# xiaoyi018/VAE-Var

Hardware: AMD Instinct MI355X
Metric: 4D-Var inner-loop iters/sec + wall-clock to convergence, 69ch 128×256 state (higher is better)
Workload: dtype f32 (GEMMs: fp16x3 split, fp32-level error)

## Files before the change

include/vaevar.h:

```cpp
#ifndef VAEVAR_H
#define VAEVAR_H
#include <stdint.h>

#ifdef __cplusplus
extern "C" {
#endif

#define VV_E_ARG 1001
#define VV_E_STATE 1002
#define VV_E_ALLOC 1003

typedef struct vv_ctx vv_ctx;

#define VV_ARCH_LGUNET 0
#define VV_ARCH_LGUNET1 1

typedef struct vv_lgunet_config {
  int img_size[2];
  int patch_size[2];
  int stride[2];
  int n_groups;
  int inchans[8];
  int outchans[8];
  int enc_dim;
// ... 150 lines not shown
int vv_profile_start(vv_ctx* ctx);
int vv_profile_stop(vv_ctx* ctx, double* ms, double* flops, double* bytes, int* launches, int ncls);

int vv_nearest_map(int in_size, int out_size, int* map);

#define VV_GEMM_F32 0
#define VV_GEMM_SPLIT 1
#define VV_GEMM_SPLIT16 2
int vv_set_gemm_math(vv_ctx* ctx, int math);
int vv_get_gemm_math(vv_ctx* ctx, int* math);

int vv_set_tuning(vv_ctx* ctx, const char* key, int value);
int vv_get_tuning(vv_ctx* ctx, const char* key, int* value);
int vv_set_debug_sync(int enable);

int vv_gemm_register_weight(vv_ctx* ctx, const float* B, int N, int K);

int vv_attention_global(vv_ctx* ctx, const float* qkv, float* out, int N, int C, int heads, void* stream);

int vv_gemm(vv_ctx* ctx, int M, int N, int K, const float* A, const float* B, const float* bias, float* C,
            int tile, void* stream);
int vv_gemm_epi(vv_ctx* ctx, int M, int N, int K, const float* A, const float* B, const float* bias, float* C,
                float* aux, int epi, int tile, void* stream);
int vv_gelu_eval(vv_ctx* ctx, const float* x, float* y, float* dy, int64_t n, int form, void* stream);

#ifdef __cplusplus
}
#endif
#endif
```

vae-var_amd/csrc/vv_engine.hip:

```cpp
#include <hip/hip_runtime.h>

#include <sys/prctl.h>
#include <time.h>

#include <algorithm>
#include <array>
#include <atomic>
#include <chrono>
#include <cmath>
#include <cstdarg>
#include <cstdio>
#include <cstdlib>
#include <cstring>
#include <memory>
#include <optional>
#include <string>
#include <unordered_map>
#include <vector>

#include "../../include/vaevar.h"
#include "vv_api.h"
#include "vv_fcst.h"
#include "vv_kernels.h"

// ... 909 lines not shown
  l.gamma = g.gamma;
  l.eps = ln.eps;
  l.pl = g.pl;
  l.rs = g.rs;
  l.stats = g.stats;
  if (bwd) {
    l.bwd = 1;
    l.lmap = ln.map;
    l.x = g.x;
    l.res = g.res;
    l.y = g.y;
  } else {
    l.gmap = ln.map;
    l.ginv = ginv;
    l.lo_x = ln.map ? 0 : 1;
    l.beta = g.beta;
  }
  return vv::gemm_ln_applies(a, l, sc.ws);
}

int gemm_layernorm(const GemmArgs& a, const LnArgs& ln, bool bwd, const int* ginv, const Scratch& sc, hipStream_t st) {
  vv::GemmLnArgs l;
  if (fixup_ln_applies(a, ln, bwd, ginv, sc, l)) {
    CK(vv::gemm_ln(a, l, st, sc.ws));
    return 0;
  }
  CK(gemm_nt(a, st, -1, sc.ws));
  CK(bwd ? layernorm_bwd(ln, st) : layernorm_fwd(ln, st));
  return 0;
}

int gemm_into_block(const GemmArgs& a, const Blk* n, const Scratch& sc, hipStream_t st, bool& ln1_ran) {
  ln1_ran = n && !ablk_fused(n->S, sc, n->ws, false);
  if (!ln1_ran) {
    CK(gemm_nt(a, st, -1, sc.ws));
    return 0;
  }
  const int* ginv = vv::tuning_of(sc.tune).fixup_ln_rows ? n->idxinv() : nullptr;
  return gemm_layernorm(a, block_ln(*n, 1, qkv_gemm(*n).apre != nullptr), false, ginv, sc, st);
}

int attn_half_fwd(const Blk& k, bool ln1_ran, const LnArgs* ln2, hipStream_t st) {
  const Scratch& sc = k.sc;
  vv::AblkArgs aa;
  if (ablk_fused(k.S, sc, k.ws, false) && ablk_args(k, nullptr, aa)) {
    CK(vv::ablk_fwd(aa, st));
// ... 849 lines not shown
        g.exec = nullptr;
        g.eager_only = true;
        (void)hipGetLastError();
        (void)fail(r ? r : (int)(ec != hipSuccess ? ec : ei), "closure graph capture failed (%s); eager launches",
                   hipGetErrorString(ec != hipSuccess ? ec : ei));
        const int r2 = closure_enqueue(ctx, P.Z, gz, nullptr, st);
        if (r2) return r2;
      }
    }
    if (g.exec) {
      VV_HIP(hipGraphLaunch(g.exec, st));
      ++g.launches;
    }
  }
  if (grad_z) VV_HIP(hipMemcpyAsync(grad_z, P.GZ, P.zn * sizeof(float), hipMemcpyDeviceToDevice, st));
  if (d_J) VV_HIP(hipMemcpyAsync(d_J, P.dJ, 2 * P.B * sizeof(double), hipMemcpyDeviceToDevice, st));
  return 0;
}

}

extern "C" {

int vv_version(void) { return 113; }

int vv_last_error(char* buf, int cap) {
  if (!buf || cap <= 0) return VV_E_ARG;
  snprintf(buf, cap, "%s", g_err.c_str());
  return 0;
}

int vv_lgunet_param_count(const vv_lgunet_config* cfg, int* count) {
  if (cfg && cfg->arch == VV_ARCH_LGUNET1) {
    std::vector<vvf::ParamInfo> v;
    std::string err;
    const int r = vvf::params(cfg, v, err);
    if (r) return fail(r, "%s", err.c_str());
    *count = (int)v.size();
    return 0;
  }
  Cfg c;
  int r = parse_cfg(cfg, c);
  if (r) return r;
  *count = (int)enumerate_params(c).size();
  return 0;
}

// ... 773 lines not shown
  if (!f) return fail(VV_E_ARG, "unknown tuning key '%s'", key ? key : "(null)");
  *value = *f;
  return 0;
}

int vv_set_debug_sync(int enable) {
  g_sync_check.store(enable ? 1 : 0, std::memory_order_relaxed);
  return 0;
}

int vv_set_closure_graph(vv_ctx* ctx, int enable) {
  if (!ctx) return fail(VV_E_ARG, "null context");
  int r = set_dev(ctx);
  if (r) return r;
  drop_graphs(ctx);
  memo_clear(ctx);
  ctx->use_graphs = enable != 0;
  return 0;
}

int vv_get_counter(const char* name, long long* value) {
  if (!name || !value) return fail(VV_E_ARG, "null argument");
  static const char* names[vv::CNT_N] = {"rowsplit", "fixup_ln", "splitk_fixup", "gather_scales", "h5_split",
                                          "closure_recall_hit", "closure_recall_miss"};
  for (int c = 0; c < vv::CNT_N; ++c)
    if (!strcmp(name, names[c])) {
      *value = vv::launch_count(c);
      return 0;
    }
  return fail(VV_E_ARG, "unknown counter '%s'", name);
}

int vv_get_closure_graph(vv_ctx* ctx, int kind, long long* info) {
  if (!ctx || !info || kind < 0 || kind > 1) return fail(VV_E_ARG, "null context / info or kind not 0 / 1");
  const auto& g = ctx->graphs[kind];
  info[0] = ctx->use_graphs ? 1 : 0;
  info[1] = g.exec ? 1 : 0;
  info[2] = g.eager_only ? 1 : 0;
  info[3] = g.launches;
  return 0;
}

int vv_get_gemm_math(vv_ctx* ctx, int* math) {
  if (!ctx || !math) return fail(VV_E_ARG, "null argument");
  *math = ctx->math;
  return 0;
}
// ... 86 lines not shown
  if (epi != EPI_STORE && epi != EPI_GELU && epi != EPI_DGELU) return fail(VV_E_ARG, "epilogue %d", epi);
  if (epi == EPI_DGELU && !aux) return fail(VV_E_ARG, "EPI_DGELU reads the pre-activation aux");
  int r = set_dev(ctx);
  if (r) return r;
  GemmArgs a = vv::gemm_args(M, N, K, 1, epi, ctx->math, &ctx->tune);
  a.g[0] = {A, nullptr, B, bias, C, nullptr, aux};
  if (ctx->math == vv::GEMM_SPLIT16) {
    VV_HIP(grow(ctx->apl, ctx->apl_halfs, (size_t)M * 2 * K, sizeof(unsigned short), (hipStream_t)stream, true));
    a.apl = ctx->apl;
    a.apl_halfs = ctx->apl_halfs;
  }
  VV_HIP(vv::gemm_nt(a, (hipStream_t)stream, tile, ctx->gemm_ws));
  return 0;
}

int vv_gemm(vv_ctx* ctx, int M, int N, int K, const float* A, const float* B, const float* bias, float* C, int tile,
            void* stream) {
  return gemm_entry(ctx, M, N, K, A, B, bias, C, nullptr, EPI_STORE, tile, stream);
}

int vv_gemm_epi(vv_ctx* ctx, int M, int N, int K, const float* A, const float* B, const float* bias, float* C,
                float* aux, int epi, int tile, void* stream) {
  return gemm_entry(ctx, M, N, K, A, B, bias, C, aux, epi, tile, stream);
}

int vv_gelu_eval(vv_ctx* ctx, const float* x, float* y, float* dy, int64_t n, int form, void* stream) {
  if (!ctx || !x || !y || !dy || n < 0 || (form != 0 && form != 1)) return fail(VV_E_ARG, "bad argument");
  int r = set_dev(ctx);
  if (r) return r;
  VV_HIP(vv::gelu_eval(x, y, dy, n, form, (hipStream_t)stream));
  return 0;
}

int vv_attention_global(vv_ctx* ctx, const float* qkv, float* out, int N, int C, int heads, void* stream) {
  if (!ctx || !qkv || !out) return fail(VV_E_ARG, "null argument");
  if (N <= 0 || !vv::gattn_supported(C, heads))
    return fail(VV_E_ARG, "global attention needs N > 0 and head_dim 64, 96, 128 or 192 (N %d, C %d, heads %d)", N, C,
                heads);
  int r = set_dev(ctx);
  if (r) return r;
  VV_HIP(grow(ctx->gattn_ws, ctx->gattn_bytes, vv::gattn_ws_bytes(N, C, heads), 1, (hipStream_t)stream, true));
  VV_HIP(vv::gattn(qkv, out, C, N, C, heads, ctx->gattn_ws, (hipStream_t)stream, ctx->tune.gattn_qf));
  return 0;
}

int vv_sc4dvar_bind(vv_ctx* ctx, int flow_model_id, int T, int C, int Hs, int Ws, const float* xb, const float* yo,
// ... 148 lines not shown
```

vae-var_amd/csrc/vv_gemm.hip:

```cpp
#include "vv_gelu.h"
#include "vv_kernels.h"
#include "vv_lanes.h"

#include <algorithm>
#include <cmath>
#include <cstdlib>
#include <cstring>
#include <mutex>
#include <type_traits>
#include <utility>
#include <vector>

namespace vv {

typedef float f4 __attribute__((ext_vector_type(4)));
typedef float f16v __attribute__((ext_vector_type(16)));

__device__ __forceinline__ float gelu_f(float x) { return gelu_fast(x); }
__device__ __forceinline__ float dgelu_f(float x) { return dgelu_fast(x); }

constexpr int KALIGN = 32;

hipError_t set_lds_limit(const void* k, size_t lds) {
  static std::mutex mu;
// ... 7 lines not shown
  done.emplace_back(k, dev);
  return hipSuccess;
}

int device_cus() {
  static std::mutex mu;
  static int cus[64] = {0};
  int dev = 0;
  if (hipGetDevice(&dev) != hipSuccess || dev < 0 || dev >= 64) return 256;
  std::lock_guard<std::mutex> lk(mu);
  if (!cus[dev]) {
    hipDeviceProp_t p;
    cus[dev] = (hipGetDeviceProperties(&p, dev) == hipSuccess && p.multiProcessorCount > 0) ? p.multiProcessorCount : 256;
  }
  return cus[dev];
}

struct TileShape {
  int id, bm, bn, wm, wn;
};
constexpr TileShape kTiles[] = {{0, 128, 128, 2, 2},  {2, 64, 64, 2, 2},    {4, 32, 64, 1, 2},    {24, 64, 64, 2, 2},
                                {25, 128, 64, 2, 2},  {26, 64, 64, 2, 2},   {27, 64, 64, 2, 2},   {34, 128, 128, 2, 2},
                                {36, 128, 128, 2, 2}, {44, 256, 128, 4, 2}, {46, 128, 128, 2, 2}, {47, 256, 128, 4, 2},
                                {48, 256, 128, 4, 2}, {49, 256, 144, 4, 2}};
constexpr const TileShape* tile_shape(int t) {
  for (const TileShape& s : kTiles)
    if (s.id == t) return &s;
  return nullptr;
}
bool valid_tile(int t) { return tile_shape(t) != nullptr; }

struct LaunchPlan {
  int T, tail;
  dim3 grid;
};
static LaunchPlan launch_plan(const GemmArgs& a, int bm, int bn) {
  const int T = ((a.N + bn - 1) / bn) * ((a.M + bm - 1) / bm);
  const int tail = a.tsplit > 1 ? T - a.tdp : 0;
  return {T, tail, dim3(tail ? a.tdp + tail * a.tsplit : T, 1, a.ngroups)};
}

template <class F>
static hipError_t with_epi(int epi, F&& f) {
  switch (epi) {
    case EPI_STORE: return f(std::integral_constant<int, EPI_STORE>{});
    case EPI_GELU: return f(std::integral_constant<int, EPI_GELU>{});
    case EPI_RESID: return f(std::integral_constant<int, EPI_RESID>{});
// ... 2056 lines not shown
static hipError_t launch_h3(const GemmArgs& a, hipStream_t s) {
  constexpr TileShape S = *tile_shape(TILE);
  constexpr int BM = S.bm;
  static_assert(S.bn == 128 && S.wm == BM / 64 && S.wn == 2, "k_gemm_h3 / k_gemm_h3m's tile");
  if (a.K % 32 || a.ksplit % 32) return hipErrorInvalidValue;
  if (!h3_ready(a)) return hipErrorInvalidValue;
  const float* sc = a.ws + kWsFloats;
  if (a.ascale_phys && !a.arow)
    sc = a.ascale;
  else if (a.ascale_phys)
    hipLaunchKernelGGL(k_gather_scales, dim3((a.M + 255) / 256, 1, a.ngroups), dim3(256), 0, s, a.ascale, a.arow,
                       const_cast<float*>(sc), a.M);
  else
    launch_rowscale(a, const_cast<float*>(sc), s);
  const size_t lds = 2 * (2 * (S.bm + S.bn) * 32) * sizeof(unsigned short);
  const LaunchPlan p = launch_plan(a, S.bm, S.bn);
  return with_epi(a.epi, [&](auto E) {
    constexpr int EPI = decltype(E)::value;
    return MF == 16 ? launch_h3m_k<EPI, BM>(a, s, p.grid, lds, p.tail, sc)
                    : launch_h3_k<EPI, BM>(a, s, p.grid, lds, p.tail, sc);
  });
}

static bool h3_tile(int t) { return t == 36 || t == 44 || t == 46 || t == 47 || t == 48 || t == 49; }
bool gemm_plane_tile(int t) { return t == 48 || t == 49; }
int* tuning_field(Tuning& t, const char* key) {
  if (!key) return nullptr;
#define VV_KNOB(name, def, ok) \
  if (!std::strcmp(key, #name)) return &t.name;
#include "vv_tuning.def"
  return nullptr;
}
bool tuning_value_ok(const char* key, int v) {
#define VV_KNOB(name, def, ok) \
  if (key && !std::strcmp(key, #name)) return ok;
#include "vv_tuning.def"
  return v == 0 || v == 1;
}

static hipError_t launch_variant(int t, const GemmArgs& a, hipStream_t s) {
  switch (t) {
    case 0: return launch_tile<0>(a, s);
    case 2: return launch_tile<2>(a, s);
    case 4: return launch_tile<4>(a, s);
    case 24: return launch_bs<24, 2>(a, s);
    case 25: return launch_bs<25, 2>(a, s);
    case 26: return launch_bs<26, 3>(a, s);
    case 27: return launch_bs<27, 1>(a, s);
    case 34: return launch_bs2(a, s);
    case 36: return launch_h3<36, 32>(a, s);
    case 44: return launch_h3<44, 32>(a, s);
    case 46: return launch_h3<46, 16>(a, s);
    case 47: return launch_h3<47, 16>(a, s);
    case 48: return launch_h4(a, s);
    case 49: return launch_h4(a, s, true);
    default: return hipErrorInvalidValue;
  }
}

static long tiles_of(const GemmArgs& a, int bm, int bn) {
  return (long)((a.M + bm - 1) / bm) * ((a.N + bn - 1) / bn) * a.ngroups;
}

struct SplitArena {
  const float* base;
  size_t n;
  const unsigned short* planes;
};
static std::vector<SplitArena> g_split;

static size_t split16_scale_off(size_t n) { return (10 * n + 255) & ~size_t(255); }
size_t split_arena_bytes(size_t n) { return split16_scale_off(n) + (n / 32 + 1) * sizeof(float); }

void register_split_arena(const float* base, size_t n, const unsigned short* planes) {
  unregister_split_arena(base);
  g_split.push_back({base, n, planes});
}
void unregister_split_arena(const float* base) {
// ... 106 lines not shown
  if (tiles_of(a, 64, 64) >= 512) return 2;
  return 4;
}

static int group_m(const GemmArgs& a, const TileShape& sh) {
  const int ntm = (a.M + sh.bm - 1) / sh.bm, ntn = (a.N + sh.bn - 1) / sh.bn;
  const double tx = (double)ntm * ntn / 8.0;
  return std::max(1, std::min(ntm, (int)std::lround(std::sqrt(tx * sh.bn / sh.bm))));
}

static int resolve_tile(GemmArgs& a, int tile_hint) {
  int t = tile_hint >= 0 ? tile_hint : pick_tile(a);
  if (!valid_tile(t)) return -1;
  const Tuning& TU = tuning_of(a.tune);
  if (tile_hint < 0 && TU.h4 && a.math == GEMM_SPLIT16 &&
      (t == 44 || t == 47 || (t == 36 && tiles_of(a, 256, 128) >= (TU.h4_small ? 64 : 144))))
    t = 48;
  for (int g = 0; g < a.ngroups; ++g) {
    a.g[g].Bh = nullptr;
    a.g[g].Bs = nullptr;
    if (h3_tile(t) && (!a.ldb || a.ldb == a.K)) split16_of(a.g[g].B, a.K, a.g[g].Bh, a.g[g].Bs);
  }
  if (h3_tile(t) && !h3_ready(a)) t = 34;
  if ((t == 48 || t == 49) && !h4_ready(a)) t = 47;
  if (t == 48 && tile_hint < 0 && TU.h5 && a.N % 144 == 0) {
    const long P = device_cus(), t48 = tiles_of(a, 256, 128), t49 = tiles_of(a, 256, 144);
    if (t48 % P != 0 && t49 % P == 0) t = 49;
  }
  return t;
}

int gemm_tile_of(const GemmArgs& a_in, int tile_hint) {
  GemmArgs a = a_in;
  if (!a.ws) a.ws = reinterpret_cast<float*>(1);
  return resolve_tile(a, tile_hint);
}

static hipError_t gemm_prepare(GemmArgs& a, int tile_hint, float* ws, int& t) {
  if (a.M <= 0 || a.N <= 0 || a.ngroups <= 0 || a.ngroups > kMaxGroups) return hipErrorInvalidValue;
  if (a.K % KALIGN != 0 || a.ksplit % KALIGN != 0 || a.ksplit <= 0 || a.ksplit > a.K) return hipErrorInvalidValue;
  if ((a.lda & 3) || (a.lda2 & 3) || (a.K & 3) || (a.ldb & 3) || (a.ldb && a.ldb < a.K)) return hipErrorInvalidValue;
  if (a.apre && (!a.ascale || a.g[0].A2)) return hipErrorInvalidValue;
  const int num_cu = device_cus();
  a.tdp = 0;
  a.tsplit = 1;
  a.ws = ws;
  a.ascale_phys = 0;
  const Tuning& TU = tuning_of(a.tune);
  if (a.ascale && TU.ln_scales) {
    bool ok = true;
    for (int g = 0; g < a.ngroups; ++g) ok = ok && !a.g[g].A2;
    a.ascale_phys = ok ? 1 : 0;
  }
  t = resolve_tile(a, tile_hint);
  if (t < 0) return hipErrorInvalidValue;
  if (a.apre && !gemm_plane_tile(t)) return hipErrorInvalidValue;
  if (a.opl && (!gemm_plane_tile(t) || (a.epi != EPI_GELU && a.epi != EPI_DGELU) || a.ngroups != 1 || a.crow || a.N % 32 ||
                !a.ors || !a.obw))
    return hipErrorInvalidValue;
  for (int g = 0; g < a.ngroups; ++g) {
    a.g[g].Bp = (t >= 21 && (!a.ldb || a.ldb == a.K)) ? split_planes_of(a.g[g].B) : nullptr;
    a.g[g].Ap = (t >= 21 && t < 36 && !a.g[g].A2 && !a.g[g].Ap) ? split_planes_exact(a.g[g].A) : a.g[g].Ap;
  }
  const TileShape& sh = *tile_shape(t);
  a.gm = group_m(a, sh);
  if (ws && a.ngroups == 1) {
    const int T = launch_plan(a, sh.bm, sh.bn).T;
    const size_t tile_f = (size_t)sh.bm * sh.bn;
    const int P = num_cu, nkt = a.K / 32;
    const int tdp = (T / P) * P, tail = T - tdp;
    if (tdp > 0 && tail > 0 && tail <= P / 2 && t != 49) {
      const int tail_minkt = std::max(1, TU.tail_minkt);
      int S = std::min(P / tail, nkt / tail_minkt);
      while (S > 1 && (size_t)tail * S * tile_f > kWsFloats) --S;
      if (S > 1) {
        a.tdp = tdp;
        a.tsplit = S;
      }
    } else if (tdp == 0 && h3_tile(t) && t != 49 && TU.small_split) {
      const int min_kt = std::max(1, t == 48 ? TU.h4_split_minkt : TU.small_split_minkt);
      int S = std::min(((t == 36 || t == 46 ? 2 : 1) * P) / T, nkt / min_kt);
      while (S > 1 && (size_t)T * S * tile_f > kWsFloats) --S;
      if (S > 1) a.tsplit = S;
    }
  }
  return hipSuccess;
}

static bool apply_h5_split(GemmArgs& a, int& t, bool ok) {
  const TileShape& sh = *tile_shape(49);
  const long P = device_cus(), T49 = tiles_of(a, sh.bm, sh.bn);
  if (!ok || !tuning_of(a.tune).h5_split || t != 48 || a.ngroups != 1 || a.N % sh.bn != 0 || a.N % 128 != 0 ||
      T49 <= 0 || P % T49 != 0 || P / T49 < 2 || P / T49 > 4 || (size_t)P * sh.bm * sh.bn > kWsFloats ||
      a.K / 32 < P / T49)
    return false;
  t = 49;
  a.tsplit = (int)(P / T49);
  a.nofix = 1;
  a.gm = group_m(a, sh);
  return true;
}

hipError_t gemm_nt(const GemmArgs& a_in, hipStream_t s, int tile_hint, float* ws) {
  GemmArgs a = a_in;
  a.nofix = 0;
  a.t49 = 0;
  int t = -1;
  if (hipError_t e = gemm_prepare(a, tile_hint, ws, t)) return e;
  const bool fix49 = apply_h5_split(a, t, tile_hint < 0 && a.tsplit > 1 && a.tdp == 0 && !a.crow && !a.opl &&
                                              (a.epi == EPI_STORE || a.epi == EPI_RESID));
  const int ph = prof_begin(s);
  hipError_t e = launch_variant(t, a, s);
  if (e == hipSuccess && fix49) {
    count_launch(CNT_SPLITK_FIXUP);
    const dim3 grid(tiles_of(a, tile_shape(49)->bm, tile_shape(49)->bn), 2, 1);
    if (a.epi == EPI_STORE)
      hipLaunchKernelGGL((k_gemm_fixup49<EPI_STORE>), grid, dim3(512), 0, s, a);
    else
      hipLaunchKernelGGL((k_gemm_fixup49<EPI_RESID>), grid, dim3(512), 0, s, a);
    e = hipGetLastError();
  }
  const double G = a.ngroups;
  double bytes = 4.0 * G * ((double)a.M * a.K + (double)a.N * a.K + (double)a.M * a.N);
  if (a.epi == EPI_RESID || a.epi == EPI_GELU || a.epi == EPI_DGELU) bytes += 4.0 * G * (double)a.M * a.N;
  prof_end(ph, s, h3_tile(t) && h3_ready(a) ? PC_GEMM16 : PC_GEMM, 2.0 * G * a.M * a.N * a.K, bytes);
  return e;
}

static bool gemm_ln_plan(GemmArgs& a, const GemmLnArgs& l, float* ws, int& t) {
  a.nofix = 0;
  if (a.ngroups != 1 || a.opl || a.N % 4 || a.N > 1280 || !ws || !l.gamma || !l.stats) return false;
  if (!l.bwd && (a.epi != EPI_RESID || !l.beta || !l.pl || !l.rs)) return false;
  if (l.bwd && (a.epi != EPI_STORE || a.g[0].bias || a.crow || !l.x || !l.y || (l.pl && !l.rs))) return false;
  if (gemm_prepare(a, -1, ws, t) != hipSuccess) return false;
  return t == 48 && a.tsplit >= 2 && a.tsplit <= 4 && a.tdp == 0;
}

bool gemm_ln_applies(const GemmArgs& a_in, const GemmLnArgs& l, float* ws) {
  GemmArgs a = a_in;
  int t = -1;
  return gemm_ln_plan(a, l, ws, t);
}

hipError_t gemm_ln(const GemmArgs& a_in, const GemmLnArgs& l, hipStream_t s, float* ws) {
  GemmArgs a = a_in;
  int t = -1;
  if (!gemm_ln_plan(a, l, ws, t)) return hipErrorInvalidValue;
  a.nofix = 1;
  a.t49 = apply_h5_split(a, t, tuning_of(a.tune).fixup_stage && (l.bwd || l.ginv || !l.gmap)) ? 1 : 0;
  const int ph = prof_begin(s);
  hipError_t e = launch_variant(t, a, s);
  if (e == hipSuccess) e = fixup_ln_launch(a, l, s);
  prof_end(ph, s, PC_GEMM16, 2.0 * a.M * a.N * a.K,
           4.0 * ((double)a.M * a.K + (double)a.N * a.K + 3.0 * (double)a.M * a.N));
  return e;
}

}
```

vae-var_amd/csrc/vv_kernels.h:

```cpp
#pragma once
#include <hip/hip_runtime.h>
#include <cstdint>
#include <cstring>
#include <string>

namespace vv {

constexpr int kMaxGroups = 8;

struct Tuning {
#define VV_KNOB(key, def, ok) int key = def;
#include "vv_tuning.def"
};
inline const Tuning& tuning_of(const Tuning* t) {
  static const Tuning kDefaultTuning{};
  return t ? *t : kDefaultTuning;
}
int* tuning_field(Tuning& t, const char* key);
bool tuning_value_ok(const char* key, int value);

enum Epi : int {
  EPI_STORE = 0,
  EPI_GELU = 1,
  EPI_RESID = 2,
// ... 75 lines not shown
size_t gattn_ws_bytes(int N, int C, int heads);
hipError_t gattn(const float* qkv, float* out, int ldo, int N, int C, int heads, void* ws, hipStream_t st,
                 int qf_per_wave = 1);

hipError_t gemm_nt(const GemmArgs& a, hipStream_t s, int tile_hint = -1, float* ws = nullptr);

struct GemmLnArgs {
  const int* gmap;
  const int* ginv;
  int lo_x;
  const float* gamma;
  const float* beta;
  float eps;
  unsigned short* pl;
  float* rs;
  float* stats;
  int bwd;
  const int* lmap;
  const float* x;
  const float* res;
  float* y;
};
bool gemm_ln_applies(const GemmArgs& a, const GemmLnArgs& l, float* ws);
hipError_t gemm_ln(const GemmArgs& a, const GemmLnArgs& l, hipStream_t s, float* ws);
hipError_t fixup_ln_launch(const GemmArgs& a, const GemmLnArgs& l, hipStream_t s);
int gemm_tile_of(const GemmArgs& a, int tile_hint = -1);
size_t gemm_ws_floats();

enum GemmMath : int { GEMM_F32 = 0, GEMM_SPLIT = 1, GEMM_SPLIT16 = 2 };
bool valid_tile(int t);
size_t split_arena_bytes(size_t n);
void register_split_arena(const float* base, size_t n, const unsigned short* planes);
void unregister_split_arena(const float* base);
hipError_t split_registered(const float* W, size_t n, int K, hipStream_t s);
hipError_t absmax(const float* x, size_t n, float* out, hipStream_t s);
hipError_t split_planes(const float* src, unsigned short* dst, size_t n, int K, hipStream_t s);

enum LnMode : int {
  LN_ROWMAP = 0,
  LN_MERGE = 1,
  LN_EXPAND = 2,
};

struct LnGroup {
  const float* x;
  const float* gamma;
  const float* beta;
  float* y;
  float* stats;
// ... 405 lines not shown
hipError_t vec_absmax_d(const float* x, int64_t n, float* partial, int nblk, double* out, hipStream_t s);
hipError_t vec_abssum(const float* x, int64_t n, double* partial, int nblk, double* out, hipStream_t s);
struct ReduceReqs {
  static constexpr int kMax = 8;
  const float* a[kMax];
  const float* b[kMax];
  int op[kMax];
};
hipError_t reduce_multi(const ReduceReqs& r, int count, int64_t n, double* partial, int nblk, double* out,
                        const double* extra, int n_extra, hipStream_t s);
hipError_t lbfgs_two_loop(float* q, const float* const* S, const float* const* Y, const float* ro, int m, float H_diag,
                          int64_t n, double* partial, int nblk, float* al, hipStream_t s);
hipError_t adam_step(float* p, const float* g, float* m, float* v, int64_t n, float lr, float b1, float b2,
                     float eps, float bc1, float bc2_sqrt, hipStream_t s);
enum ProfClass : int { PC_GEMM = 0, PC_ATTN = 1, PC_LN = 2, PC_PATCH = 3, PC_MISFIT = 4, PC_VEC = 5, PC_GEMM16 = 6,
                       PC_TOWER = 7, PC_N = 8 };
int prof_begin(hipStream_t s);
void prof_end(int h, hipStream_t s, int cls, double flops, double bytes);
void prof_enable(bool on);
bool prof_enabled();
void prof_read(double* ms, double* flops, double* bytes, int* n);
enum Counter : int { CNT_ROWSPLIT = 0, CNT_FIXUP_LN = 1, CNT_SPLITK_FIXUP = 2, CNT_GATHER_SCALES = 3, CNT_H5_SPLIT = 4,
                     CNT_RECALL_HIT = 5, CNT_RECALL_MISS = 6,
                     CNT_N = 7 };
void count_launch(int c);
long long launch_count(int c);

hipError_t transpose2d(const float* in, float* out, int rows, int cols, hipStream_t s);

struct MlpGroup {
  const float* x;
  const float *gamma, *beta;
  float* stats;
  const unsigned short* w1h;
  const float* w1s;
  const float* b1;
  const unsigned short* w2h;
  const float* w2s;
  const float* b2;
  float* h1;
  const float* dy;
  float* out;
  float* rs;
};
struct MlpArgs {
  int M, C, ngroups;
  int hc;
// ... 56 lines not shown
```

vae-var_amd/vaevar/_lib.py:

```python
from __future__ import annotations

import ctypes
import os

HERE = os.path.dirname(os.path.abspath(__file__))
LIB_PATH = os.environ.get("VAEVAR_LIB", os.path.join(HERE, "libvaevar.so"))

c_int, c_int64, c_float, c_double, c_void_p, c_char_p = (ctypes.c_int, ctypes.c_int64, ctypes.c_float,
                                                          ctypes.c_double, ctypes.c_void_p, ctypes.c_char_p)
P = ctypes.POINTER


class VVConfig(ctypes.Structure):
    _fields_ = [
        ("img_size", c_int * 2),
        ("patch_size", c_int * 2),
        ("stride", c_int * 2),
        ("n_groups", c_int),
        ("inchans", c_int * 8),
        ("outchans", c_int * 8),
        ("enc_dim", c_int),
        ("embed_dim", c_int),
        ("window_size", c_int),
        ("n_enc_levels", c_int),
# ... 104 lines not shown
    "vv_axpby": (c_int, [c_void_p, c_void_p, c_void_p, c_float, c_void_p, c_float, c_int64, c_void_p]),
    "vv_scale": (c_int, [c_void_p, c_void_p, c_float, c_int64, c_void_p]),
    "vv_copy": (c_int, [c_void_p, c_void_p, c_void_p, c_int64, c_void_p]),
    "vv_lbfgs_two_loop": (c_int, [c_void_p, c_void_p, P(c_void_p), P(c_void_p), P(c_float), c_int, c_float, c_int64,
                                  c_void_p]),
    "vv_adam": (c_int, [c_void_p, c_void_p, c_void_p, c_void_p, c_void_p, c_int64, c_float, c_float, c_float,
                        c_float, c_int, c_void_p]),
    "vv_profile_start": (c_int, [c_void_p]),
    "vv_profile_stop": (c_int, [c_void_p, P(c_double), P(c_double), P(c_double), P(c_int), c_int]),
    "vv_nearest_map": (c_int, [c_int, c_int, P(c_int)]),
    "vv_set_gemm_math": (c_int, [c_void_p, c_int]),
    "vv_set_closure_graph": (c_int, [c_void_p, c_int]),
    "vv_get_closure_graph": (c_int, [c_void_p, c_int, P(ctypes.c_longlong)]),
    "vv_get_counter": (c_int, [ctypes.c_char_p, P(ctypes.c_longlong)]),
    "vv_integrate": (c_int, [c_void_p, c_int, c_void_p, c_void_p, c_int, c_int, c_int, c_void_p, c_void_p,
                             c_int, c_void_p]),
    "vv_get_gemm_math": (c_int, [c_void_p, P(c_int)]),
    "vv_set_tuning": (c_int, [c_void_p, ctypes.c_char_p, c_int]),
    "vv_get_tuning": (c_int, [c_void_p, ctypes.c_char_p, P(c_int)]),
    "vv_set_debug_sync": (c_int, [c_int]),
    "vv_attention_global": (c_int, [c_void_p, c_void_p, c_void_p, c_int, c_int, c_int, c_void_p]),
    "vv_gemm_register_weight": (c_int, [c_void_p, c_void_p, c_int, c_int]),
    "vv_gemm": (c_int, [c_void_p, c_int, c_int, c_int, c_void_p, c_void_p, c_void_p, c_void_p, c_int, c_void_p]),
    "vv_gemm_epi": (c_int, [c_void_p, c_int, c_int, c_int, c_void_p, c_void_p, c_void_p, c_void_p, c_void_p, c_int,
                            c_int, c_void_p]),
    "vv_gelu_eval": (c_int, [c_void_p, c_void_p, c_void_p, c_void_p, c_int64, c_int, c_void_p]),
    "vv_sc4dvar_bind": (c_int, [c_void_p, c_int, c_int, c_int, c_int, c_int, c_void_p, c_void_p, c_void_p, c_void_p,
                                c_void_p, c_void_p, c_float, c_void_p, c_int, P(c_double), P(c_double), c_int,
                                P(c_double), P(c_double), P(c_double), c_double, c_int]),
    "vv_sc4dvar_closure": (c_int, [c_void_p, c_void_p, c_void_p, P(c_double), P(c_double), c_void_p]),
    "vv_sc4dvar_transform": (c_int, [c_void_p, c_void_p, c_void_p, c_void_p]),
    "vv_resample_nearest": (c_int, [c_void_p, c_void_p, c_void_p, c_int, c_int, c_int, c_int, c_int, c_int, c_void_p]),
}

EXPORTED = sorted(_SIGS)


class VVError(RuntimeError):
    pass


def _load():
    if not os.path.exists(LIB_PATH):
        raise ImportError(f"libvaevar.so not found at {LIB_PATH}: build it with `make -C vae-var_amd/csrc` "
                          "(or __graft_entry__.build()); there is no CPU fallback")
    import torch
# ... 42 lines not shown
```

vae-var_amd/vaevar/engine.py:

```python
from __future__ import annotations

import ctypes
import os

import numpy as np
import torch

from . import _lib
from ._lib import VVConfig, check, lib


def _ptr(t: torch.Tensor):
    if not t.is_cuda:
        raise ValueError("libvaevar compute entry points take device tensors")
    if t.dtype != torch.float32 or not t.is_contiguous():
        raise ValueError("expected a contiguous float32 tensor")
    return ctypes.c_void_p(t.data_ptr())


def _stream(stream=None):
    if stream is not None:
        return ctypes.c_void_p(stream.cuda_stream)
    return ctypes.c_void_p(torch._C._cuda_getCurrentRawStream(torch._C._cuda_getDevice()))


class Context:

    _by_dev: dict = {}

    TUNING_KEYS = ("h3_mink", "h3_big", "h3_mf16", "small_split", "small_split_minkt", "tail_minkt", "ln_scales",
                   "win_attn", "h4", "ln_planes", "gattn", "gattn_qf", "h4_small", "h4_split_minkt",
                   "win_mfma", "fc_h3_mink", "fuse_mlp", "fuse_attn", "attn_mfma", "gelu_planes", "attn_planes", "fixup_ln", "h5", "fc_conv_mf",
                   "mlp_hc", "h4_gather", "fixup_ln_rows", "grid_fused", "fixup_stage", "host_wait", "h5_split",
                   "patch_pers", "bs_tile", "fixup_ln_cross")

    def __init__(self, device: int = 0):
        self.device = device
        self.h = ctypes.c_void_p()
        env = os.environ
        math = env.get("VAEVAR_GEMM_MATH") or None
        if math is not None and math not in self.GEMM_MATH:
            raise ValueError(f"VAEVAR_GEMM_MATH={math!r}: expected one of {sorted(self.GEMM_MATH)}")
        tuning = {}
        for k in self.TUNING_KEYS:
            v = env.get("VAEVAR_" + k.upper())
            if v is not None and v != "":
                try:
                    tuning[k] = int(v)
                except ValueError:
                    raise ValueError(f"VAEVAR_{k.upper()}={v!r} is not an integer") from None
        check(lib.vv_ctx_create(device, ctypes.byref(self.h)), "ctx_create")
        try:
            if math is not None:
                self.gemm_math = math
            if env.get("VAEVAR_GRAPH", "1")[:1] == "0":
                self.set_closure_graph(False)
            if env.get("VAEVAR_SYNC_CHECK", "0")[:1] == "1":
# ... 137 lines not shown
        check(lib.vv_get_closure_graph(self.h, kind, info), "get_closure_graph")
        return {"enabled": bool(info[0]), "instantiated": bool(info[1]), "eager_only": bool(info[2]),
                "launches": int(info[3])}

    def attention_global(self, qkv, heads: int):
        if not (qkv.is_cuda and qkv.dtype == torch.float32 and qkv.dim() == 2 and qkv.is_contiguous()):
            raise ValueError("qkv must be a contiguous 2-D float32 CUDA tensor [N, 3C] (row stride 3C)")
        N, C3 = qkv.shape
        if C3 % 3 or (C3 // 3) % heads:
            raise ValueError(f"qkv width {C3} is not 3C with C divisible by heads={heads}")
        out = torch.empty(N, C3 // 3, device=qkv.device, dtype=torch.float32)
        check(lib.vv_attention_global(self.h, _ptr(qkv), _ptr(out), N, C3 // 3, heads, _stream()), "attention_global")
        return out

    def gemm_register_weight(self, B):
        check(lib.vv_gemm_register_weight(self.h, _ptr(B), B.shape[0], B.shape[1]), "gemm_register_weight")

    def gemm(self, A, B, bias=None, tile=-1):
        M, K = A.shape
        N = B.shape[0]
        C = torch.empty(M, N, device=A.device, dtype=torch.float32)
        bp = _ptr(bias) if bias is not None else None
        check(lib.vv_gemm(self.h, M, N, K, _ptr(A), _ptr(B), bp, _ptr(C), tile, _stream()), "gemm")
        return C

    EPI = {"store": 0, "gelu": 1, "dgelu": 3}

    def gemm_epi(self, A, B, epi, aux=None, bias=None, tile=-1):
        M, K = A.shape
        N = B.shape[0]
        C = torch.empty(M, N, device=A.device, dtype=torch.float32)
        bp = _ptr(bias) if bias is not None else None
        ap = _ptr(aux) if aux is not None else None
        check(lib.vv_gemm_epi(self.h, M, N, K, _ptr(A), _ptr(B), bp, _ptr(C), ap, self.EPI[epi], tile, _stream()),
              "gemm_epi")
        return C

    def gelu_eval(self, x, form=0):
        y, dy = torch.empty_like(x), torch.empty_like(x)
        check(lib.vv_gelu_eval(self.h, _ptr(x), _ptr(y), _ptr(dy), x.numel(), form, _stream()), "gelu_eval")
        return y, dy


class _NetFn(torch.autograd.Function):
    @staticmethod
    def forward(ctx, x, net, slot, out_limit):
# ... 336 lines not shown
```

Before: 57.98.

## Add one-pass 64x144 fp16x3 GEMM kernel replacing split-K with fixup

```diff
diff --git a/include/vaevar.h b/include/vaevar.h
--- a/include/vaevar.h
+++ b/include/vaevar.h
@@ -196,6 +196,8 @@
             int tile, void* stream);
 int vv_gemm_epi(vv_ctx* ctx, int M, int N, int K, const float* A, const float* B, const float* bias, float* C,
                 float* aux, int epi, int tile, void* stream);
+int vv_gemm_rows(vv_ctx* ctx, int M, int N, int K, const float* A, const int* arow, const float* B, const float* bias,
+                 const float* R, float* C, int tile, void* stream);
 int vv_gelu_eval(vv_ctx* ctx, const float* x, float* y, float* dy, int64_t n, int form, void* stream);
 
 #ifdef __cplusplus
diff --git a/vae-var_amd/csrc/vv_engine.hip b/vae-var_amd/csrc/vv_engine.hip
--- a/vae-var_amd/csrc/vv_engine.hip
+++ b/vae-var_amd/csrc/vv_engine.hip
@@ -955,6 +955,11 @@
 int gemm_layernorm(const GemmArgs& a, const LnArgs& ln, bool bwd, const int* ginv, const Scratch& sc, hipStream_t st) {
   vv::GemmLnArgs l;
   if (fixup_ln_applies(a, ln, bwd, ginv, sc, l)) {
+    if (vv::gemm_ln_onepass(a, l, sc.ws)) {
+      CK(gemm_nt(a, st, 51, sc.ws));
+      CK(layernorm_fwd(ln, st));
+      return 0;
+    }
     CK(vv::gemm_ln(a, l, st, sc.ws));
     return 0;
   }
@@ -1850,7 +1855,7 @@
 
 extern "C" {
 
-int vv_version(void) { return 113; }
+int vv_version(void) { return 114; }
 
 int vv_last_error(char* buf, int cap) {
   if (!buf || cap <= 0) return VV_E_ARG;
@@ -2670,7 +2675,7 @@
 int vv_get_counter(const char* name, long long* value) {
   if (!name || !value) return fail(VV_E_ARG, "null argument");
   static const char* names[vv::CNT_N] = {"rowsplit", "fixup_ln", "splitk_fixup", "gather_scales", "h5_split",
-                                          "closure_recall_hit", "closure_recall_miss"};
+                                          "closure_recall_hit", "closure_recall_miss", "onepass"};
   for (int c = 0; c < vv::CNT_N; ++c)
     if (!strcmp(name, names[c])) {
       *value = vv::launch_count(c);
@@ -2803,6 +2808,33 @@
 int vv_gemm_epi(vv_ctx* ctx, int M, int N, int K, const float* A, const float* B, const float* bias, float* C,
                 float* aux, int epi, int tile, void* stream) {
   return gemm_entry(ctx, M, N, K, A, B, bias, C, aux, epi, tile, stream);
+}
+
+int vv_gemm_rows(vv_ctx* ctx, int M, int N, int K, const float* A, const int* arow, const float* B, const float* bias,
+                 const float* R, float* C, int tile, void* stream) {
+  if (!ctx || !A || !B || !C) return fail(VV_E_ARG, "null argument");
+  if (tile >= 0 && !vv::valid_tile(tile)) return fail(VV_E_ARG, "tile hint %d is not a library kernel", tile);
+  if (M <= 0 || N <= 0 || K <= 0 || K % 32) return fail(VV_E_ARG, "bad GEMM shape %dx%dx%d (K a multiple of 32)", M, N, K);
+  if (ctx->math != vv::GEMM_SPLIT16) return fail(VV_E_STATE, "vv_gemm_rows needs the fp16x3 math");
+  int r = set_dev(ctx);
+  if (r) return r;
+  hipStream_t st = (hipStream_t)stream;
+  GemmArgs a = vv::gemm_args(M, N, K, 1, R ? EPI_RESID : EPI_STORE, ctx->math, &ctx->tune);
+  a.g[0] = {A, nullptr, B, bias, C, R, nullptr};
+  const size_t halfs = (size_t)M * 2 * K;
+  VV_HIP(grow(ctx->apl, ctx->apl_halfs, halfs + 2 * (size_t)M, sizeof(unsigned short), st, true));
+  if (arow) {
+    float* rs = reinterpret_cast<float*>(ctx->apl + halfs);
+    VV_HIP(vv::rowsplit(a, rs, ctx->apl, st));
+    a.arow = arow;
+    a.apre = ctx->apl;
+    a.ascale = rs;
+  } else {
+    a.apl = ctx->apl;
+    a.apl_halfs = halfs;
+  }
+  VV_HIP(vv::gemm_nt(a, st, tile, ctx->gemm_ws));
+  return 0;
 }
 
 int vv_gelu_eval(vv_ctx* ctx, const float* x, float* y, float* dy, int64_t n, int form, void* stream) {
diff --git a/vae-var_amd/csrc/vv_gemm.hip b/vae-var_amd/csrc/vv_gemm.hip
--- a/vae-var_amd/csrc/vv_gemm.hip
+++ b/vae-var_amd/csrc/vv_gemm.hip
@@ -53,7 +53,7 @@
 constexpr TileShape kTiles[] = {{0, 128, 128, 2, 2},  {2, 64, 64, 2, 2},    {4, 32, 64, 1, 2},    {24, 64, 64, 2, 2},
                                 {25, 128, 64, 2, 2},  {26, 64, 64, 2, 2},   {27, 64, 64, 2, 2},   {34, 128, 128, 2, 2},
                                 {36, 128, 128, 2, 2}, {44, 256, 128, 4, 2}, {46, 128, 128, 2, 2}, {47, 256, 128, 4, 2},
-                                {48, 256, 128, 4, 2}, {49, 256, 144, 4, 2}};
+                                {48, 256, 128, 4, 2}, {49, 256, 144, 4, 2}, {51, 64, 144, 2, 2}};
 constexpr const TileShape* tile_shape(int t) {
   for (const TileShape& s : kTiles)
     if (s.id == t) return &s;
@@ -2156,8 +2156,8 @@
   });
 }
 
-static bool h3_tile(int t) { return t == 36 || t == 44 || t == 46 || t == 47 || t == 48 || t == 49; }
-bool gemm_plane_tile(int t) { return t == 48 || t == 49; }
+static bool h3_tile(int t) { return t == 36 || t == 44 || t == 46 || t == 47 || t == 48 || t == 49 || t == 51; }
+bool gemm_plane_tile(int t) { return t == 48 || t == 49 || t == 51; }
 int* tuning_field(Tuning& t, const char* key) {
   if (!key) return nullptr;
 #define VV_KNOB(name, def, ok) \
@@ -2171,6 +2171,8 @@
 #include "vv_tuning.def"
   return v == 0 || v == 1;
 }
+
+static hipError_t launch_h6(const GemmArgs& a, hipStream_t s);
 
 static hipError_t launch_variant(int t, const GemmArgs& a, hipStream_t s) {
   switch (t) {
@@ -2188,6 +2190,7 @@
     case 47: return launch_h3<47, 16>(a, s);
     case 48: return launch_h4(a, s);
     case 49: return launch_h4(a, s, true);
+    case 51: return launch_h6(a, s);
     default: return hipErrorInvalidValue;
   }
 }
@@ -2340,7 +2343,7 @@
     if (h3_tile(t) && (!a.ldb || a.ldb == a.K)) split16_of(a.g[g].B, a.K, a.g[g].Bh, a.g[g].Bs);
   }
   if (h3_tile(t) && !h3_ready(a)) t = 34;
-  if ((t == 48 || t == 49) && !h4_ready(a)) t = 47;
+  if (gemm_plane_tile(t) && !h4_ready(a)) t = 47;
   if (t == 48 && tile_hint < 0 && TU.h5 && a.N % 144 == 0) {
     const long P = device_cus(), t48 = tiles_of(a, 256, 128), t49 = tiles_of(a, 256, 144);
     if (t48 % P != 0 && t49 % P == 0) t = 49;
@@ -2387,7 +2390,7 @@
     const size_t tile_f = (size_t)sh.bm * sh.bn;
     const int P = num_cu, nkt = a.K / 32;
     const int tdp = (T / P) * P, tail = T - tdp;
-    if (tdp > 0 && tail > 0 && tail <= P / 2 && t != 49) {
+    if (tdp > 0 && tail > 0 && tail <= P / 2 && t != 49 && t != 51) {
       const int tail_minkt = std::max(1, TU.tail_minkt);
       int S = std::min(P / tail, nkt / tail_minkt);
       while (S > 1 && (size_t)tail * S * tile_f > kWsFloats) --S;
@@ -2395,7 +2398,7 @@
         a.tdp = tdp;
         a.tsplit = S;
       }
-    } else if (tdp == 0 && h3_tile(t) && t != 49 && TU.small_split) {
+    } else if (tdp == 0 && h3_tile(t) && t != 49 && t != 51 && TU.small_split) {
       const int min_kt = std::max(1, t == 48 ? TU.h4_split_minkt : TU.small_split_minkt);
       int S = std::min(((t == 36 || t == 46 ? 2 : 1) * P) / T, nkt / min_kt);
       while (S > 1 && (size_t)T * S * tile_f > kWsFloats) --S;
@@ -2405,18 +2408,38 @@
   return hipSuccess;
 }
 
-static bool apply_h5_split(GemmArgs& a, int& t, bool ok) {
+static int h5_split_ways(const GemmArgs& a) {
   const TileShape& sh = *tile_shape(49);
   const long P = device_cus(), T49 = tiles_of(a, sh.bm, sh.bn);
-  if (!ok || !tuning_of(a.tune).h5_split || t != 48 || a.ngroups != 1 || a.N % sh.bn != 0 || a.N % 128 != 0 ||
-      T49 <= 0 || P % T49 != 0 || P / T49 < 2 || P / T49 > 4 || (size_t)P * sh.bm * sh.bn > kWsFloats ||
-      a.K / 32 < P / T49)
-    return false;
+  if (a.ngroups != 1 || a.N % sh.bn != 0 || a.N % 128 != 0 || T49 <= 0 || P % T49 != 0 || P / T49 < 2 ||
+      P / T49 > 4 || (size_t)P * sh.bm * sh.bn > kWsFloats || a.K / 32 < P / T49)
+    return 0;
+  return (int)(P / T49);
+}
+static bool apply_h5_split(GemmArgs& a, int& t, bool ok) {
+  const int S = ok && tuning_of(a.tune).h5_split && t == 48 ? h5_split_ways(a) : 0;
+  if (!S) return false;
   t = 49;
-  a.tsplit = (int)(P / T49);
+  a.tsplit = S;
   a.nofix = 1;
-  a.gm = group_m(a, sh);
+  a.gm = group_m(a, *tile_shape(49));
   return true;
+}
+
+constexpr int kOnepassMaxK = 1152;
+static bool onepass_shape(const GemmArgs& a) {
+  const TileShape& sh = *tile_shape(51);
+  return a.M % sh.bm == 0 && a.N % sh.bn == 0 && a.ngroups == 1 && !a.opl &&
+         (a.epi == EPI_STORE || a.epi == EPI_RESID) && !(a.apre && a.arow && !tuning_of(a.tune).h4_gather);
+}
+static bool onepass_ok(const GemmArgs& a) {
+  return tuning_of(a.tune).onepass && a.K <= kOnepassMaxK && onepass_shape(a);
+}
+static void apply_onepass(GemmArgs& a, int& t) {
+  t = 51;
+  a.nofix = 0;
+  a.t49 = 0;
+  a.gm = group_m(a, *tile_shape(51));
 }
 
 hipError_t gemm_nt(const GemmArgs& a_in, hipStream_t s, int tile_hint, float* ws) {
@@ -2425,8 +2448,17 @@
   a.t49 = 0;
   int t = -1;
   if (hipError_t e = gemm_prepare(a, tile_hint, ws, t)) return e;
-  const bool fix49 = apply_h5_split(a, t, tile_hint < 0 && a.tsplit > 1 && a.tdp == 0 && !a.crow && !a.opl &&
-                                              (a.epi == EPI_STORE || a.epi == EPI_RESID));
+  bool fix49 = apply_h5_split(a, t, tile_hint < 0 && a.tsplit > 1 && a.tdp == 0 && !a.crow && !a.opl &&
+                                        (a.epi == EPI_STORE || a.epi == EPI_RESID));
+  if (tile_hint == 51) {
+    const int S = h5_split_ways(a);
+    if (t != 51 || !S || !onepass_shape(a)) return hipErrorInvalidValue;
+    a.tdp = 0;
+    a.tsplit = S;
+  } else if (fix49 && onepass_ok(a)) {
+    apply_onepass(a, t);
+    fix49 = false;
+  }
   const int ph = prof_begin(s);
   hipError_t e = launch_variant(t, a, s);
   if (e == hipSuccess && fix49) {
@@ -2460,12 +2492,22 @@
   return gemm_ln_plan(a, l, ws, t);
 }
 
+static bool gemm_ln_h5_split(GemmArgs& a, const GemmLnArgs& l, int& t) {
+  return apply_h5_split(a, t, tuning_of(a.tune).fixup_stage && (l.bwd || l.ginv || !l.gmap));
+}
+
+bool gemm_ln_onepass(const GemmArgs& a_in, const GemmLnArgs& l, float* ws) {
+  GemmArgs a = a_in;
+  int t = -1;
+  return !l.bwd && gemm_ln_plan(a, l, ws, t) && gemm_ln_h5_split(a, l, t) && onepass_ok(a);
+}
+
 hipError_t gemm_ln(const GemmArgs& a_in, const GemmLnArgs& l, hipStream_t s, float* ws) {
   GemmArgs a = a_in;
   int t = -1;
   if (!gemm_ln_plan(a, l, ws, t)) return hipErrorInvalidValue;
   a.nofix = 1;
-  a.t49 = apply_h5_split(a, t, tuning_of(a.tune).fixup_stage && (l.bwd || l.ginv || !l.gmap)) ? 1 : 0;
+  a.t49 = gemm_ln_h5_split(a, l, t) ? 1 : 0;
   const int ph = prof_begin(s);
   hipError_t e = launch_variant(t, a, s);
   if (e == hipSuccess) e = fixup_ln_launch(a, l, s);
@@ -2474,4 +2516,214 @@
   return e;
 }
 
-}
+constexpr int kH6Stages = 6;
+
+template <bool ACCUM>
+__device__ __forceinline__ float h6_fold(float run, float acc, float sc) {
+#pragma clang fp contract(off)
+  const float p = acc * sc;
+  return ACCUM ? run + p : p;
+}
+
+template <int EPI, bool AG, int TN>
+__device__ __forceinline__ void h6_body(const GemmArgs& args, const float* __restrict__ rs,
+                                        const unsigned short* __restrict__ apl, int wave, int lane) {
+  constexpr int BM = 64, BN = 144, BK = 32, TM = 2, NSTG = kH6Stages, AHEAD = NSTG - 1, NP = 7;
+  constexpr int STG = (BM + BN) * 2 * BK;
+  typedef float accv __attribute__((ext_vector_type(4)));
+  extern __shared__ __attribute__((aligned(16))) unsigned short lds16[];
+  const int wm = wave >> 1, wn = wave & 1;
+  const GemmGroup G = args.g[0];
+  const int M = args.M, N = args.N, K = args.K, S = args.tsplit, nk = K / BK;
+  const int ntn = N / BN, ntm = M / BM;
+  int mb, nb;
+  tile_mn(xcd_remap(blockIdx.x, ntm * ntn), ntm, ntn, mb, nb, args.gm);
+  const int m0 = mb * BM, n0 = nb * BN;
+
+  const int prow = lane >> 3, pslot = lane & 7;
+  const unsigned short* src[NP];
+#pragma unroll
+  for (int j = 0; j < NP; ++j) {
+    const int p = min(wave + 4 * j, 25), row = 8 * (j < 2 ? p : p - 8) + prow;
+    if (j < 2) {
+      int gr = min(m0 + row, M - 1);
+      if (args.apre && args.arow) gr = args.arow[gr];
+      src[j] = apl + (size_t)gr * 2 * K + 8 * (pslot ^ ((row >> 1) & 7));
+    } else {
+      const int gn = min(n0 + row, N - 1);
+      src[j] = G.Bh + (size_t)gn * 2 * K + 8 * (pslot ^ ((row >> 1) & 7));
+    }
+  }
+  auto piece = [&](int kt, int buf, int j) {
+    __builtin_amdgcn_global_load_lds((const void*)(src[j] + 2 * kt * BK),
+                                     (lds_ptr_t)(lds16 + buf * STG + min(wave + 4 * j, 25) * 8 * 64), 16, 0, 0);
+  };
+
+  const int rin = lane & 15, hh = lane >> 4;
+  const int ck0 = (hh ^ ((rin >> 1) & 7)) * 8, ck1 = ((4 + hh) ^ ((rin >> 1) & 7)) * 8;
+  const int aoff = (wm * TM * 16 + rin) * 64, boff = (BM + wn * 80 + rin) * 64;
+  auto read_a = [&](int buf, int a, h8v (&fa)[TM][2]) {
+    const unsigned short* Sb = lds16 + buf * STG + aoff + a * 16 * 64;
+    fa[a][1] = *reinterpret_cast<const h8v*>(Sb + ck1);
+    fa[a][0] = *reinterpret_cast<const h8v*>(Sb + ck0);
+  };
+  auto read_b = [&](int buf, int b, h8v (&fb)[TN][2]) {
+    const unsigned short* Sb = lds16 + buf * STG + boff + b * 16 * 64;
+    fb[b][0] = *reinterpret_cast<const h8v*>(Sb + ck0);
+    fb[b][1] = *reinterpret_cast<const h8v*>(Sb + ck1);
+  };
+
+  accv acc[TM][5], run[TM][5];
+#pragma unroll
+  for (int a = 0; a < TM; ++a)
+#pragma unroll
+    for (int b = 0; b < 5; ++b)
+#pragma unroll
+      for (int r = 0; r < 4; ++r) acc[a][b][r] = run[a][b][r] = 0.0f;
+
+  auto step = [&](int t, const h8v (&fa)[TM][2], const h8v (&fb)[TN][2], h8v (&na)[TM][2], h8v (&nb_)[TN][2]) {
+    const int rb = (t + 1) % NSTG, sb = (t + AHEAD) % NSTG, sk = min(t + AHEAD, nk - 1);
+    asm volatile("s_waitcnt vmcnt(%0) lgkmcnt(0)" ::"n"((AHEAD - 2) * NP) : "memory");
+    __builtin_amdgcn_sched_barrier(0);
+    __builtin_amdgcn_s_barrier();
+    __builtin_amdgcn_sched_barrier(0);
+#pragma unroll
+    for (int b = 0; b < TN; ++b) {
+#pragma unroll
+      for (int a = 0; a < TM; ++a) acc[a][b] = __builtin_amdgcn_mfma_f32_16x16x32_f16(fa[a][1], fb[b][0], acc[a][b], 0, 0, 0);
+#pragma unroll
+      for (int a = 0; a < TM; ++a) acc[a][b] = __builtin_amdgcn_mfma_f32_16x16x32_f16(fa[a][0], fb[b][1], acc[a][b], 0, 0, 0);
+#pragma unroll
+      for (int a = 0; a < TM; ++a) acc[a][b] = __builtin_amdgcn_mfma_f32_16x16x32_f16(fa[a][0], fb[b][0], acc[a][b], 0, 0, 0);
+      __builtin_amdgcn_sched_barrier(0);
+      if (b < TM) read_a(rb, b, na);
+      read_b(rb, b, nb_);
+#pragma unroll
+      for (int j = b; j < NP; j += TN) piece(sk, sb, j);
+      __builtin_amdgcn_sched_barrier(0);
+    }
+  };
+
+#pragma unroll
+  for (int q = 0; q < 2; ++q)
+#pragma unroll
+    for (int j = 0; j < NP; ++j) piece(min(q, nk - 1), q, j);
+  float ia[TM][4], sbv[TN];
+#pragma unroll
+  for (int a = 0; a < TM; ++a)
+#pragma unroll
+    for (int r = 0; r < 4; ++r) {
+      const int row = min(m0 + wm * TM * 16 + a * 16 + 4 * hh + r, M - 1);
+      ia[a][r] = __uint_as_float((254u << 23) - __float_as_uint(rs[AG ? args.arow[row] : row]));
+    }
+#pragma unroll
+  for (int b = 0; b < TN; ++b) sbv[b] = G.Bs[(size_t)min(n0 + wn * 80 + b * 16 + rin, N - 1) * (K / 32)];
+  asm volatile("s_waitcnt vmcnt(0)" ::: "memory");
+  __builtin_amdgcn_sched_barrier(0);
+#pragma unroll
+  for (int q = 2; q < AHEAD; ++q)
+#pragma unroll
+    for (int j = 0; j < NP; ++j) piece(min(q, nk - 1), q, j);
+  __builtin_amdgcn_s_barrier();
+  __builtin_amdgcn_sched_barrier(0);
+  h8v fa0[TM][2], fb0[TN][2], fa1[TM][2], fb1[TN][2];
+#pragma unroll
+  for (int a = 0; a < TM; ++a) read_a(0, a, fa0);
+#pragma unroll
+  for (int b = 0; b < TN; ++b) read_b(0, b, fb0);
+  __builtin_amdgcn_sched_barrier(0);
+
+  int c = 0, kend = nk / S;
+  auto chunk_end = [&](int t) {
+    if (t + 1 != kend) return;
+#pragma unroll
+    for (int a = 0; a < TM; ++a)
+#pragma unroll
+      for (int b = 0; b < TN; ++b)
+#pragma unroll
+        for (int r = 0; r < 4; ++r) {
+          const float sc = ia[a][r] * sbv[b];
+          run[a][b][r] = c == 0 ? h6_fold<false>(run[a][b][r], acc[a][b][r], sc)
+                                : h6_fold<true>(run[a][b][r], acc[a][b][r], sc);
+          acc[a][b][r] = 0.0f;
+        }
+    ++c;
+    kend = ((c + 1) * nk) / S;
+  };
+  int t = 0;
+  for (; t + 1 < nk; t += 2) {
+    step(t, fa0, fb0, fa1, fb1);
+    chunk_end(t);
+    step(t + 1, fa1, fb1, fa0, fb0);
+    chunk_end(t + 1);
+  }
+  if (t < nk) {
+    step(t, fa0, fb0, fa1, fb1);
+    chunk_end(t);
+  }
+  asm volatile("s_waitcnt vmcnt(0) lgkmcnt(0)" ::: "memory");
+
+  epilogue<32, 16 * TN, 1, 1, EPI, 16, true>(args, G, run, m0 + wm * 32, n0 + wn * 80, 0, 0, rin, hh);
+}
+
+template <int EPI, bool AG>
+__global__ __launch_bounds__(256, 1) void k_gemm_h6(GemmArgs args, const float* __restrict__ ascale,
+                                                    const unsigned short* __restrict__ apl) {
+  const int lane = threadIdx.x & 63, wave = __builtin_amdgcn_readfirstlane(threadIdx.x >> 6);
+  if (wave & 1)
+    h6_body<EPI, AG, 4>(args, ascale, apl, wave, lane);
+  else
+    h6_body<EPI, AG, 5>(args, ascale, apl, wave, lane);
+}
+
+template <int EPI, bool AG>
+static hipError_t launch_h6_k(const GemmArgs& a, hipStream_t s, dim3 grid, size_t lds, const float* sc,
+                              const unsigned short* planes) {
+  if (hipError_t e = set_lds_limit((const void*)k_gemm_h6<EPI, AG>, lds)) return e;
+  hipLaunchKernelGGL((k_gemm_h6<EPI, AG>), grid, dim3(256), lds, s, a, sc, planes);
+  return hipGetLastError();
+}
+
+hipError_t rowsplit(const GemmArgs& a, float* rs, unsigned short* pl, hipStream_t s) {
+  if (a.M <= 0 || a.K <= 0 || a.K % 32 || a.K > 4608 || !rs || !pl) return hipErrorInvalidValue;
+  const int nv = (a.K + 255) / 256;
+  const dim3 grid((a.M + 3) / 4, 1, a.ngroups);
+  count_launch(CNT_ROWSPLIT);
+  switch (nv <= 5 ? 5 : nv <= 9 ? 9 : nv <= 14 ? 14 : 18) {
+    case 5: hipLaunchKernelGGL(k_rowsplit<5>, grid, dim3(256), 0, s, a, rs, pl); break;
+    case 9: hipLaunchKernelGGL(k_rowsplit<9>, grid, dim3(256), 0, s, a, rs, pl); break;
+    case 14: hipLaunchKernelGGL(k_rowsplit<14>, grid, dim3(256), 0, s, a, rs, pl); break;
+    default: hipLaunchKernelGGL(k_rowsplit<18>, grid, dim3(256), 0, s, a, rs, pl); break;
+  }
+  return hipGetLastError();
+}
+
+static hipError_t launch_h6(const GemmArgs& a, hipStream_t s) {
+  constexpr TileShape S51 = *tile_shape(51);
+  static_assert(S51.bm == 64 && S51.bn == 144 && S51.wm == 2 && S51.wn == 2, "k_gemm_h6's tile");
+  if (a.K % 32 || a.ksplit % 32 || !h3_ready(a) || !h4_ready(a) || !onepass_shape(a)) return hipErrorInvalidValue;
+  if (a.tdp || a.tsplit < 2 || a.tsplit > 4 || a.K / 32 < a.tsplit || a.nofix) return hipErrorInvalidValue;
+  float* sc = a.ws + kWsFloats;
+  const unsigned short* planes = a.apl;
+  bool agather = false;
+  if (a.apre) {
+    planes = a.apre;
+    sc = const_cast<float*>(a.ascale);
+    agather = a.arow != nullptr;
+  } else if (hipError_t e = rowsplit(a, sc, a.apl, s)) {
+    return e;
+  }
+  GemmArgs b = a;
+  b.escale = sc;
+  b.agather = agather ? 1 : 0;
+  const size_t lds = kH6Stages * (2 * (S51.bm + S51.bn) * 32) * sizeof(unsigned short);
+  const dim3 grid((a.M / S51.bm) * (a.N / S51.bn), 1, 1);
+  count_launch(CNT_ONEPASS);
+  if (a.epi == EPI_STORE)
+    return agather ? launch_h6_k<EPI_STORE, true>(b, s, grid, lds, sc, planes)
+                   : launch_h6_k<EPI_STORE, false>(b, s, grid, lds, sc, planes);
+  return agather ? launch_h6_k<EPI_RESID, true>(b, s, grid, lds, sc, planes)
+                 : launch_h6_k<EPI_RESID, false>(b, s, grid, lds, sc, planes);
+}
+
+}
diff --git a/vae-var_amd/csrc/vv_kernels.h b/vae-var_amd/csrc/vv_kernels.h
--- a/vae-var_amd/csrc/vv_kernels.h
+++ b/vae-var_amd/csrc/vv_kernels.h
@@ -121,9 +121,11 @@
   float* y;
 };
 bool gemm_ln_applies(const GemmArgs& a, const GemmLnArgs& l, float* ws);
+bool gemm_ln_onepass(const GemmArgs& a, const GemmLnArgs& l, float* ws);
 hipError_t gemm_ln(const GemmArgs& a, const GemmLnArgs& l, hipStream_t s, float* ws);
 hipError_t fixup_ln_launch(const GemmArgs& a, const GemmLnArgs& l, hipStream_t s);
 int gemm_tile_of(const GemmArgs& a, int tile_hint = -1);
+hipError_t rowsplit(const GemmArgs& a, float* rs, unsigned short* pl, hipStream_t s);
 size_t gemm_ws_floats();
 
 enum GemmMath : int { GEMM_F32 = 0, GEMM_SPLIT = 1, GEMM_SPLIT16 = 2 };
@@ -575,7 +577,8 @@
 void prof_read(double* ms, double* flops, double* bytes, int* n);
 enum Counter : int { CNT_ROWSPLIT = 0, CNT_FIXUP_LN = 1, CNT_SPLITK_FIXUP = 2, CNT_GATHER_SCALES = 3, CNT_H5_SPLIT = 4,
                      CNT_RECALL_HIT = 5, CNT_RECALL_MISS = 6,
-                     CNT_N = 7 };
+                     CNT_ONEPASS = 7,
+                     CNT_N = 8 };
 void count_launch(int c);
 long long launch_count(int c);
 
diff --git a/vae-var_amd/vaevar/_lib.py b/vae-var_amd/vaevar/_lib.py
--- a/vae-var_amd/vaevar/_lib.py
+++ b/vae-var_amd/vaevar/_lib.py
@@ -150,6 +150,8 @@
     "vv_attention_global": (c_int, [c_void_p, c_void_p, c_void_p, c_int, c_int, c_int, c_void_p]),
     "vv_gemm_register_weight": (c_int, [c_void_p, c_void_p, c_int, c_int]),
     "vv_gemm": (c_int, [c_void_p, c_int, c_int, c_int, c_void_p, c_void_p, c_void_p, c_void_p, c_int, c_void_p]),
+    "vv_gemm_rows": (c_int, [c_void_p, c_int, c_int, c_int, c_void_p, c_void_p, c_void_p, c_void_p, c_void_p, c_void_p,
+                             c_int, c_void_p]),
     "vv_gemm_epi": (c_int, [c_void_p, c_int, c_int, c_int, c_void_p, c_void_p, c_void_p, c_void_p, c_void_p, c_int,
                             c_int, c_void_p]),
     "vv_gelu_eval": (c_int, [c_void_p, c_void_p, c_void_p, c_void_p, c_int64, c_int, c_void_p]),
diff --git a/vae-var_amd/vaevar/engine.py b/vae-var_amd/vaevar/engine.py
--- a/vae-var_amd/vaevar/engine.py
+++ b/vae-var_amd/vaevar/engine.py
@@ -32,7 +32,7 @@
                    "win_attn", "h4", "ln_planes", "gattn", "gattn_qf", "h4_small", "h4_split_minkt",
                    "win_mfma", "fc_h3_mink", "fuse_mlp", "fuse_attn", "attn_mfma", "gelu_planes", "attn_planes", "fixup_ln", "h5", "fc_conv_mf",
                    "mlp_hc", "h4_gather", "fixup_ln_rows", "grid_fused", "fixup_stage", "host_wait", "h5_split",
-                   "patch_pers", "bs_tile", "fixup_ln_cross")
+                   "patch_pers", "bs_tile", "fixup_ln_cross", "onepass")
 
     def __init__(self, device: int = 0):
         self.device = device
@@ -216,6 +216,20 @@
         C = torch.empty(M, N, device=A.device, dtype=torch.float32)
         bp = _ptr(bias) if bias is not None else None
         check(lib.vv_gemm(self.h, M, N, K, _ptr(A), _ptr(B), bp, _ptr(C), tile, _stream()), "gemm")
+        return C
+
+    def gemm_rows(self, A, B, arow=None, bias=None, resid=None, tile=-1):
+        M, K = A.shape
+        N = B.shape[0]
+        C = torch.empty(M, N, device=A.device, dtype=torch.float32)
+        opt = lambda t: _ptr(t) if t is not None else None
+        rows = None
+        if arow is not None:
+            if not (arow.is_cuda and arow.dtype == torch.int32 and arow.is_contiguous() and arow.numel() == M):
+                raise ValueError("arow must be a contiguous int32 CUDA tensor of M rows")
+            rows = ctypes.c_void_p(arow.data_ptr())
+        check(lib.vv_gemm_rows(self.h, M, N, K, _ptr(A), rows, _ptr(B), opt(bias), opt(resid), _ptr(C), tile,
+                               _stream()), "gemm_rows")
         return C
 
     EPI = {"store": 0, "gelu": 1, "dgelu": 3}
```

Result: slower. 57.31 (-1.2%).
